# yhtang/GraphDot

Measured on AMD Instinct MI355X. Metric: graph-pairs/sec (Gram matrix), higher is better.
Workload: dtype f64

## Files before the change

graphdot_amd/csrc/device/mgk_oc.h:

```cpp
#ifndef GRAPHDOT_HIP_MGK_OC_H_
#define GRAPHDOT_HIP_MGK_OC_H_
#include "mgk_solver.h"

#ifdef GD_MARKS
#define GD_MARK(name) asm volatile("; GDMARK " #name)
#else
#define GD_MARK(name) ((void)0)
#endif

namespace graphdot {
namespace mgk {

template<int DMAX> struct class_order {
    constexpr static int NC = DMAX + 1, NCP = NC * NC;
    unsigned char d1[NCP], d2[NCP];
    constexpr class_order() : d1{}, d2{} {
        int n = 0;
        for (int p = DMAX * DMAX; p >= 0; --p)
            for (int a = 0; a <= DMAX; ++a)
                for (int b = 0; b <= DMAX; ++b)
                    if (a * b == p) {
                        d1[n] = (unsigned char)a;
                        d2[n] = (unsigned char)b;
                        ++n;
// ... 137 lines not shown
    constexpr static bool PK2 = DENSE && packed_edge<EdgeK>::value && sizeof(real) == 4;
    constexpr static int NR = R * T;
    constexpr static int NC = DMAX + 1;
    constexpr static int NCP = NC * NC;
    constexpr static int NTAB = ((NCP + 63) / 64) * 64;
    constexpr static int NM = S > 0 ? (S + 31) / 32 : 1;
    constexpr static int SETUP_CHUNK = 4;
    constexpr static bool ONE_PASS = sizeof(real) == 4 || W == 1;
    constexpr static int GCH = (STATIC && W == 1 && !NODAL && (sizeof(real) == 8 || C == 2)) ? 16 : 8;
    constexpr static bool ADDTID = W == 1 && C == 1 && sizeof(real) == 4 && !STATIC && !FLY;
    constexpr static bool PACK = C == 1 && !NODAL && !STATIC && !FLY &&
                                 (sizeof(real) == 4 ? (S >= 64 && W >= 8) : W >= 16);
    constexpr static int NADR = PACK ? (S + 1) / 2 : SA;
    constexpr static int lds_slot_count() {
        if (C != 1 || NODAL || NGRAD || STATIC || FLY || W == 1) return 0;
        if (sizeof(real) == 8 && W == 16 && (S == 40 || S == 64)) return 10;
        return 0;
    }
    constexpr static int SL = lds_slot_count();
    constexpr static int SREG = S - SL;
    constexpr static bool SEQ = C == 2 && STATIC && !NODAL && W == 1 && sizeof(real) == 8;
    constexpr static int CW = SEQ ? 1 : C;
    constexpr static bool LEAN = STATIC && C == 2 && !NODAL && !SEQ;
#ifndef GD_OC_FSCAL
#define GD_OC_FSCAL 1
#endif
    constexpr static bool FSCAL = GD_OC_FSCAL != 0 && sizeof(real) == 8 && !NGRAD;
    using sreal = std::conditional_t<FSCAL, float, real>;
    constexpr static int NSYS = C / CW;
    constexpr static bool DLDS = sizeof(real) == 8 && STATIC && W == 1 && C == 1 && !NODAL &&
                                 !NGRAD && !MAXIMIN && !FLY && R == 6;
    constexpr static bool HAS_Y = (!STATIC && !FLY) || LEAN || SEQ || DLDS;
    constexpr static int Y_REALS = DLDS ? 2 * R * 64 * W : R * 64 * W * C;
    template<class L> constexpr static int grid_slots() {
        if constexpr (L::is_static && !NGRAD) return L::T.end[0] == DMAX * DMAX ? DMAX * DMAX : 0;
        else return 0;
    }
    constexpr static int G0 = grid_slots<LAY>();
    static_assert(G0 == 0 || ONE_PASS, "the grid walk belongs to the one-pass slot setup");
    template<class L> constexpr static bool layout_matches() {
        if constexpr (L::is_static) return L::S == S && L::R == R;
        else return true;
    }
    static_assert(layout_matches<LAY>(), "the static layout must have S slots in R batches");
    template<class M> __device__ static __forceinline__ bool flush_at(int s, M const &m) {
        if constexpr (STATIC) return LAY::T.last[s];
        else return (m[s / 32] >> (s % 32)) & 1u;
    }
    constexpr static bool KEEP_X = NODAL || C == 2;
    constexpr static int n_jac = PStart::jac_dims + 1 + NodeK::jac_dims + EdgeK::jac_dims;
    constexpr static int off_q = PStart::jac_dims;
    constexpr static int off_v = off_q + 1;
    constexpr static int off_e = off_v + NodeK::jac_dims;
    constexpr static class_order<DMAX> ORD{};

    struct lds_t {
        real red[2][2 * W];
        int tab_off[NTAB];
        int tab_cls[64];
        unsigned mm_cell[4];
    };

    __device__ static __forceinline__ int uni(int v) { return __builtin_amdgcn_readfirstlane(v); }

    template<class V> __device__ static __forceinline__ V scalar_load(V const *ptr) {
        static_assert(sizeof(V) % 4 == 0, "whole dwords");
        typedef const unsigned __attribute__((address_space(4))) *const_words;
        const_words w = (const_words)(std::uintptr_t)ptr;
        unsigned buf[sizeof(V) / 4];
#pragma unroll
        for (unsigned k = 0; k < sizeof(V) / 4; ++k) buf[k] = w[k];
// ... 2 lines not shown
        return out;
    }

    __device__ static __forceinline__ graph_header_t load_header(graph_header_t const *ptr, [[maybe_unused]] int &n_orig) {
        if constexpr (QUOT) {
            graph_header_t h = scalar_load(ptr);
            n_orig = (int)((unsigned)h.n_node >> 16);
            h.n_node &= 0xFFFF;
            return h;
        } else {
            return scalar_load(ptr);
        }
    }
    __device__ static __forceinline__ Graph view_graph(char const *image, graph_header_t const &h, [[maybe_unused]] int n_orig) {
        if constexpr (QUOT) return Graph::quotient(image, h, n_orig);
        else return Graph(image, h);
    }

    __device__ static __forceinline__ float cg_ratio(float a, float b) { return a / b; }
    __device__ static __forceinline__ double cg_ratio(double a, double b) {
        double y = __builtin_amdgcn_rcp(b);
        y = __builtin_fma(__builtin_fma(-b, y, 1.0), y, y);
        y = __builtin_fma(__builtin_fma(-b, y, 1.0), y, y);
        return a * y;
    }

    __device__ static __forceinline__ int row_pos(int k, int wv, int lane) {
        return k * T + 64 * ((k & 1) ? W - 1 - wv : wv) + lane;
    }

    struct row_t {
        int i1, i2, rs1, rs2, d1, d2, prod;
    };
    constexpr static int GD_ = G0 ? DMAX : 1;
    constexpr static int GQ_ = QUOT ? GD_ : 1;
    struct grid_t {
        unsigned a[GD_], b[GD_];
        unsigned j1[GD_], j2[GD_];
        unsigned t1[GD_], t2[GD_];
        bool u[GD_], v[GD_];
        int row;
    };

    __device__ static __forceinline__ void run(PF const &full, lds_t &lds, real *dyn) {
        P const &prm = common(full);
        const int lane = wave::laneid();
        const int tid = (W == 1) ? lane : (int)threadIdx.x;
        const int wv = (W == 1) ? 0 : uni((int)(threadIdx.x / 64));
        real *const lp = dyn;
        real *const lY = lp + (size_t)prm.u_capacity * C;
        unsigned *const rowmap = reinterpret_cast<unsigned *>(lY + (HAS_Y ? (size_t)Y_REALS : (size_t)0));
        char *const lG1 = reinterpret_cast<char *>(rowmap + NR);
        char *const lG2 = lG1 + prm.g_capacity;
        [[maybe_unused]] real *const lV = reinterpret_cast<real *>(lG2 + prm.g_capacity);
        real *const red0 = lds.red[0], *const red1 = lds.red[1];
        using reduce = alternating_reduce<real, W>;
        using sreduce = alternating_reduce<sreal, W>;
        sreal *const sred0 = reinterpret_cast<sreal *>(red0), *const sred1 = reinterpret_cast<sreal *>(red1);
        const unsigned lY_off = uni((int)lds_offset(lY));
        graph_header_t const *const headers = reinterpret_cast<graph_header_t const *>(prm.arena);
        const int dump = (int)prm.u_capacity - 1;

        if constexpr (DENSE) {
            if (prm.flags & F_DENSE) {
                for (unsigned k = tid; k < prm.u_capacity * (unsigned)C; k += T) lp[k] = real(0);
                job_sync<W>();
            }
        }
        for (unsigned t = blockIdx.x; t < prm.n_launch_jobs; t += gridDim.x) {
            const job_t job = scalar_load(prm.jobs + t);
            [[maybe_unused]] int no1 = 0, no2 = 0;
            const graph_header_t h1 = load_header(headers + job.i, no1), h2 = load_header(headers + job.j, no2);
            const int n1 = h1.n_node, n2 = h2.n_node, N = n1 * n2;
            const int ldp = n2 | 1;
            const real q = prm.q, q0 = prm.q0;
            const real inv1q2 = real(1) / ((real(1) - q) * (real(1) - q));
            const real bscale = q * q / (q0 * q0);
            const unsigned nzpad1 = ((unsigned)n1 + 3u) & ~3u, nzpad2 = ((unsigned)n2 + 3u) & ~3u;
            const unsigned cb1 = TAB ? (nzpad1 + (((unsigned)h1.n_nz + 3u) & ~3u) + 15u) & ~15u : 0u;
            const unsigned cb2 = TAB ? (nzpad2 + (((unsigned)h2.n_nz + 3u) & ~3u) + 15u) & ~15u : 0u;

            GD_MARK(stage);
            job_sync<W>();
            {
                typedef unsigned v4 __attribute__((ext_vector_type(4)));
                const unsigned w1 = (h1.perm + 2u * n1 - h1.degree + cb1 + 15u) / 16u;
                const unsigned w2 = (h2.perm + 2u * n2 - h2.degree + cb2 + 15u) / 16u;
                const v4 *const s1 = reinterpret_cast<const v4 *>(prm.arena + h1.degree - cb1);
                const v4 *const s2 = reinterpret_cast<const v4 *>(prm.arena + h2.degree - cb2);
                v4 *const d1 = reinterpret_cast<v4 *>(lG1);
                v4 *const d2 = reinterpret_cast<v4 *>(lG2);
                constexpr int K = 2;
                const unsigned wmax = w1 > w2 ? w1 : w2;
#pragma nounroll
                for (unsigned base = 0; base < wmax; base += K * T) {
                    v4 v1[K], v2[K];
#pragma unroll
                    for (int k = 0; k < K; ++k) {
                        const unsigned w = base + k * T + tid;
                        v1[k] = w < w1 ? s1[w] : v4{0u, 0u, 0u, 0u};
                        v2[k] = w < w2 ? s2[w] : v4{0u, 0u, 0u, 0u};
                    }
#pragma unroll
                    for (int k = 0; k < K; ++k) {
                        const unsigned w = base + k * T + tid;
// ... 133 lines not shown

            struct walk_t {
                unsigned e1, end1, last1, e2, rs2, end2;
                int row;
                __device__ __forceinline__ bool valid() const { return e1 < end1; }
                __device__ __forceinline__ unsigned a() const { return e1 < last1 ? e1 : last1; }
                __device__ __forceinline__ void next() {
                    ++e2;
                    const bool wrap = e2 == end2;
                    e2 = wrap ? rs2 : e2;
                    e1 += wrap ? 1u : 0u;
                }
            };
            auto open_walk = [&](int kb) -> walk_t {
                const row_t r = open_row(kb);
                const bool live = r.prod > 0;
                walk_t w;
                w.e1 = live ? (unsigned)r.rs1 : 0u;
                w.end1 = live ? (unsigned)(r.rs1 + r.d1) : 0u;
                w.last1 = live ? (unsigned)(r.rs1 + r.d1 - 1) : 0u;
                w.rs2 = live ? (unsigned)r.rs2 : 0u;
                w.end2 = live ? (unsigned)(r.rs2 + r.d2) : 1u;
                w.e2 = w.rs2;
                w.row = r.i1 * ldp + r.i2;
                return w;
            };

            auto open_grid = [&](unsigned base, unsigned elem) -> grid_t {
                const row_t r = open_row(0);
                const bool live = r.prod > 0;
                grid_t g;
                g.row = r.i1 * ldp + r.i2;
#pragma unroll
                for (int k = 0; k < GD_; ++k) {
                    g.u[k] = k < r.d1;
                    g.v[k] = k < r.d2;
                    g.a[k] = live ? (unsigned)r.rs1 + (g.u[k] ? (unsigned)k : 0u) : 0u;
                    g.b[k] = live ? (unsigned)r.rs2 + (g.v[k] ? (unsigned)k : 0u) : 0u;
                    const nz_t z1 = at32(g1.nz, g.a[k]), z2 = at32(g2.nz, g.b[k]);
                    g.j1[k] = base + __umul24((unsigned)z1.j, (unsigned)ldp) * elem;
                    g.j2[k] = (unsigned)z2.j * elem;
                    if constexpr (TAB) {
                        g.t1[k] = __umul24((unsigned)ecls1[g.a[k]], nec);
                        g.t2[k] = (unsigned)ecls2[g.b[k]];
                    }
                }
                return g;
            };

            GD_MARK(slots);
            real val[SA];
            unsigned adr[NADR];
            const unsigned lp_off = lds_offset(lp);
            constexpr unsigned ELEM = CW * sizeof(real);
            unsigned fm[NM];
#pragma unroll
            for (int w = 0; w < NM; ++w) fm[w] = 0;
            int n_slots = 0;
            if constexpr (!FLY) {
                if constexpr (STATIC) {
#pragma unroll
                    for (int k = 0; k < R; ++k)
                        if (k * T < N) n_slots = LAY::T.end[k];
                } else {
#pragma unroll
                for (int k = 0; k < R; ++k) {
                    const int pos = row_pos(k, wv, 0);
                    int trip = 0;
                    if (pos < N) {
                        const unsigned rm = (unsigned)uni((int)rowmap[pos]);
                        const int i1 = (int)(rm >> 16), i2 = (int)(rm & 0xFFFFu);
                        trip = uni(((int)lrp1[i1 + 1] - (int)lrp1[i1]) * ((int)lrp2[i2 + 1] - (int)lrp2[i2]));
                    }
                    if (trip > 0) {
                        n_slots += trip;
                        const int last = n_slots - 1;
#pragma unroll
                        for (int w = 0; w < NM; ++w)
                            if (last / 32 == w) fm[w] |= 1u << (last % 32);
                    }
                }
                n_slots = n_slots > S ? S : n_slots;
                }
                if constexpr (ONE_PASS) {
                    int kb = 0;
                    walk_t cur = G0 ? walk_t{} : open_walk(0);
                    [[maybe_unused]] grid_t grid;
                    [[maybe_unused]] edge_t ge1[GD_], ge2[GD_];
                    [[maybe_unused]] real gw1[GQ_], gw2[GQ_];
                    if constexpr (G0 > 0) {
                        grid = open_grid(lp_off, ELEM);
                        if constexpr (QUOT) {
#pragma unroll
                            for (int k = 0; k < GD_; ++k) {
                                gw1[k] = qweight(g1, at32(g1.nz, grid.a[k]));
                                gw2[k] = qweight(g2, at32(g2.nz, grid.b[k]));
                            }
                        }
                        if constexpr (!TAB || (GD_WEIGHTED && edge_weight<edge_t>::value)) {
#pragma unroll
                            for (int k = 0; k < GD_; ++k) {
                                ge1[k] = at32(g1.edge, grid.a[k]);
                                ge2[k] = at32(g2.edge, grid.b[k]);
                            }
                        }
                    }
    #pragma unroll
                    for (int s = 0; s < S; ++s) {
                        if (s % SETUP_CHUNK == 0) __builtin_amdgcn_sched_barrier(0);
                        real e;
                        bool ok;
                        unsigned col;
                        if (s < G0) {
                            const int gu = s / GD_, gv = s % GD_;
                            ok = grid.u[gu] && grid.v[gv];
                            if constexpr (TAB) {
                                e = at32(ketab, grid.t1[gu] + grid.t2[gv]);
                                if constexpr (GD_WEIGHTED && edge_weight<edge_t>::value)
                                    e *= real(edge_weight<edge_t>::get(ge1[gu])) *
                                         real(edge_weight<edge_t>::get(ge2[gv]));
                            } else {
                                e = prm.edge_kernel(ge1[gu], ge2[gv]);
                            }
                            if constexpr (QUOT) e *= gw1[gu] * gw2[gv];
                            col = ok ? grid.j1[gu] + grid.j2[gv] : lp_off;
                        } else {
                        ok = cur.valid();
                        const unsigned a = cur.a(), b = cur.e2;
                        const nz_t z1 = at32(g1.nz, a), z2 = at32(g2.nz, b);
                        if constexpr (TAB) {
                            e = at32(ketab, __umul24((unsigned)ecls1[a], nec) + ecls2[b]);
                            if constexpr (GD_WEIGHTED && edge_weight<edge_t>::value)
                                e *= real(edge_weight<edge_t>::get(at32(g1.edge, a))) *
                                     real(edge_weight<edge_t>::get(at32(g2.edge, b)));
                        } else {
                            const edge_t e1 = at32(g1.edge, a), e2 = at32(g2.edge, b);
                            e = prm.edge_kernel(e1, e2);
                        }
                        if constexpr (QUOT) e *= qweight(g1, z1) * qweight(g2, z2);
                        col = ok ? __umul24((unsigned)z1.j, (unsigned)ldp) + (unsigned)z2.j : 0u;
                        col = lp_off + col * ELEM;
                        }
                        if (SL > 0 && s >= SREG) {
                            lV[(s - SREG) * T + tid] = ok ? e : real(0);
                        } else {
                            val[s] = ok ? e : real(0);
                        }
// ... 1084 lines not shown
                                const unsigned col = (unsigned)at32(g2.nz, b).j;
                                real w = w1 * load_real_at<real>(rowp + col * ELEM);
                                if constexpr (TAB) {
                                    const unsigned cidx = c1 + ecls2[b];
                                    if constexpr (GD_WEIGHTED && edge_weight<edge_t>::value)
                                        w *= real(edge_weight<edge_t>::get(at32(g2.edge, b)));
#pragma unroll
                                    for (int jj = 0; jj < EdgeK::jac_dims; ++jj)
                                        jac[off_e + jj] += w * at32(dketab, (unsigned)jj * nec * nec + cidx);
                                } else {
                                    auto de = prm.edge_kernel._j_a_c_o_b_i_a_n_(e1, at32(g2.edge, b));
#pragma unroll
                                    for (int jj = 0; jj < EdgeK::jac_dims; ++jj) jac[off_e + jj] += w * real(de[jj]);
                                }
                            }
                        }
                    }
                } else if constexpr (EdgeK::jac_dims > 0) {
                    int kb = 0;
                    walk_t cur = G0 ? walk_t{} : open_walk(0);
                    [[maybe_unused]] grid_t grid;
                    if constexpr (G0 > 0) {
                        grid = open_grid(0u, 0u);
                        cur.row = grid.row;
                    }
                    auto yp_of = [&](int row) -> real {
                        if constexpr (SEQ) return lp[(unsigned)prm.u_capacity + (unsigned)row];
                        else return lp[row * 2 + 1];
                    };
                    real yrow = yp_of(cur.row);
#pragma unroll
                    for (int s = 0; s < S; ++s) {
                        if (s < n_slots) {
                            const bool ok = s < G0 ? grid.u[s / GD_] && grid.v[s % GD_] : cur.valid();
                            const unsigned a = s < G0 ? grid.a[s / GD_] : cur.a();
                            const unsigned b = s < G0 ? grid.b[s % GD_] : cur.e2;
                            real w = ok ? yrow * load_real_at<real>(adr[s]) : real(0);
                            if constexpr (TAB) {
                                const unsigned cidx = __umul24((unsigned)ecls1[a], nec) + ecls2[b];
                                if constexpr (GD_WEIGHTED && edge_weight<edge_t>::value)
                                    w *= real(edge_weight<edge_t>::get(g1.edge[a])) *
                                         real(edge_weight<edge_t>::get(g2.edge[b]));
#pragma unroll
                                for (int jj = 0; jj < EdgeK::jac_dims; ++jj)
                                    jac[off_e + jj] += w * at32(dketab, (unsigned)jj * nec * nec + cidx);
                            } else {
                                const edge_t e1 = g1.edge[a], e2 = g2.edge[b];
                                auto de = prm.edge_kernel._j_a_c_o_b_i_a_n_(e1, e2);
#pragma unroll
                                for (int jj = 0; jj < EdgeK::jac_dims; ++jj) jac[off_e + jj] += w * real(de[jj]);
                            }
                            if (s >= G0) cur.next();
                            if (flush_at(s, fm) && s != S - 1) {
                                ++kb;
                                cur = open_walk(kb);
                                yrow = yp_of(cur.row);
                            }
                        }
                    }
                }
#pragma unroll
                for (int j = 0; j < n_jac; ++j) {
                    const real g = reduce::sum(jac[j], (j & 1) ? red1 : red0);
                    if (tid == 0) {
                        if (flags & F_PACKED) {
                            prm.gradient[(size_t)prm.order[t] * n_jac + j] = g;
                        } else if (flags & F_DIAGONAL) {
                            prm.gradient[(size_t)I1 + (size_t)prm.nX * j] = g;
                        } else {
// ... 38 lines not shown
```

graphdot_amd/csrc/gdhost.cpp:

```cpp
#include "gdhost.h"
#include "gdquotient.h"

#include <algorithm>
#include <cstdlib>
#include <cstring>
#include <numeric>
#include <atomic>
#include <cmath>
#include <exception>
#include <mutex>
#include <thread>
#include <vector>

namespace {

constexpr int64_t ALIGN = 16;
inline int64_t pad(int64_t n) { return (n + ALIGN - 1) / ALIGN * ALIGN; }

struct rect_order_t {
    int a[256], b[256], prod[257];
    int n_upto[16], upto[16][256];
    rect_order_t() {
        int n = 0;
        for (int p = 15 * 15; p >= 0; --p)
// ... 418 lines not shown
        int prods[256], nr = 0;
        {
            const uint16_t *h1 = hist + (size_t)a * 16, *h2 = hist + (size_t)b * 16;
            int64_t c = 0;
            for (int u = 0; u < RECT.n_upto[pmd]; ++u) {
                const int k = RECT.upto[pmd][u];
                const int64_t sz = (int64_t)h1[RECT.a[k]] * h2[RECT.b[k]];
                if (sz == 0) continue;
                c += sz;
                cum[nr] = c;
                prods[nr] = RECT.prod[k];
                ++nr;
            }
        }
        auto trip_at = [&](int64_t first) -> int {
            if (first >= N) return 0;
            int k = 0;
            while (k < nr && cum[k] <= first) ++k;
            return k < nr ? prods[k] : 0;
        };
        int trips1[MAXL + 1];
        {
            int k = 0;
            for (int bt = 0; bt <= MAXL; ++bt) {
                const int64_t first = 64 * (int64_t)bt;
                while (k < nr && cum[k] <= first) ++k;
                trips1[bt] = (first < N && k < nr) ? prods[k] : 0;
            }
        }
        for (int32_t v = 0; v < n_var; ++v) {
            const bool fly = S[v] == 0;
            if (!fly && (pmd_true > D[v] || pmd_true > 14)) continue;
            const int64_t T = 64 * (int64_t)W[v];
            if (N > T * R[v] || np_ >= (fly ? 0x3FFF : 0xFFFF)) continue;
            const int64_t NR = T * R[v];
            const int64_t pcap = (np_ + 1 + 3) / 4 * 4;
            const int64_t NRy = ((n_L[v] > 0 && C != 2) || fly) ? 0 : NR;
            const int64_t lds = (pcap + NRy) * C * real_size + 4 * NR + 2 * gbytes +
                                4 * (int64_t)W[v] * real_size + 4 * (D[v] > 6 ? 128 : 64) + 256 + 16 +
                                (extra_lds ? extra_lds[v] : 0);
            if (lds > lds_limit) continue;
            const int64_t nb = (N + T - 1) / T;
            bool ok = true;
            if (fly) {
                ok = pmd_true > fly_min_degree;
            } else if (n_L[v] > 0) {
                for (int64_t k = 0; k < nb && ok; ++k) {
                    const int cap = k < n_L[v] && k < MAXL ? L[(size_t)v * MAXL + k] : 0;
                    ok = (W[v] == 1 && k <= MAXL ? trips1[k] : trip_at(k * T)) <= cap;
                }
            } else if (W[v] == 1 && nb <= MAXL + 1) {
                int64_t total = 0;
                for (int64_t k = 0; k < nb; ++k) total += trips1[k];
                ok = total <= S[v];
            } else {
                int64_t worst = 0;
                for (int32_t wv = 0; wv < W[v]; ++wv) {
                    int64_t total = 0;
                    for (int64_t k = 0; k < nb; ++k)
                        total += trip_at(k * T + 64 * ((k & 1) ? W[v] - 1 - wv : wv));
                    worst = std::max(worst, total);
                }
                ok = worst <= S[v];
            }
            if (ok) {
                choice[t] = v;
                break;
            }
        }
// ... 146 lines not shown
```

graphdot_amd/kernel/marginalized/_backend_hip.py:

```python
import copy
import os
import re
import uuid
import zlib
from collections import OrderedDict, namedtuple
import numpy as np
from ...codegen import Template
from ...util import gcpause
from ...util.cookie import IdentityCache
from ...codegen.sympy_printer import to_real_expr
from ...codegen.typetool import _dtype_util
from ...hip import jit, runtime
from ...microkernel import TensorProduct, Product
from ...util.iterable import flatten, fold_like
from ._backend import Backend
from ._devicegraph import (DeviceGraph, GraphArena, HIST_BINS, class_bytes,
                           degree_histograms, graph_features, pack_many,
                           quotient_graph)

_TEMPLATE = os.path.join(os.path.dirname(__file__), 'template.hip')

F_NODAL, F_DIAGONAL, F_SYMMETRIC, F_LMIN1, F_BLOCK, F_PACKED, F_REFCOMPAT, \
    F_DENSE = 1, 2, 4, 8, 16, 32, 64, 128

# ... 9 lines not shown
def stream_parts(costs, count, resident, queued):
    if costs is None or len(costs) == 0:
        return max(1, min(resident // max(count, 1), STREAM_MAX_PARTS))
    c = np.asarray(costs, dtype=np.float64)
    best, best_t = 1, max(c[0], c.sum() / max(1, min(resident, queued)))
    table = dict(STREAM_PART_EFFICIENCY)
    ms, es = zip(*STREAM_PART_EFFICIENCY)
    own = min(resident // max(len(c), 1), STREAM_MAX_PARTS)
    for M in sorted(set(ms[1:]) | ({own} if own > 1 else set())):
        if M > min(resident, STREAM_MAX_PARTS):
            break
        eff = table.get(M) or float(np.interp(np.log2(M), np.log2(ms), es))
        groups = max(1, resident // M)
        pad = -len(c) % groups
        load = np.concatenate((c, np.zeros(pad))).reshape(-1, groups).sum(0)
        t = load.max() / (M * eff)
        if t < 0.95 * best_t:
            best, best_t = M, t
    return best


def OCStatic(*L, D=4):
    return OCVariant(1, int(sum(L)), len(L), D, tuple(int(x) for x in L))


VARIANTS = [
    Variant(1, 8, 2), Variant(1, 12, 3), Variant(1, 16, 4), Variant(1, 20, 5),
    Variant(1, 24, 6), Variant(1, 28, 7), Variant(1, 32, 9), Variant(1, 48, 9),
    Variant(1, 64, 16),
    Variant(4, 16, 4), Variant(4, 32, 8), Variant(4, 64, 16),
    Variant(16, 16, 2), Variant(16, 32, 4), Variant(16, 64, 8),
    Variant(16, 128, 16),
]
OC_STATIC_VARIANTS = [
    OCStatic(16), OCStatic(16, 4), OCStatic(16, 4, 1), OCStatic(16, 4, 4),
    OCStatic(16, 4, 4, 1), OCStatic(16, 4, 4, 1, 1), OCStatic(16, 4, 4, 3, 1),
    OCStatic(16, 4, 4, 3, 1, 1), OCStatic(16, 4, 4, 4, 1, 1, 1),
    OCStatic(16, 4, 4, 4, 3, 1, 1, 1), OCStatic(16, 4, 4, 4, 4, 1, 1, 1, 1),
]
OC_FLY_VARIANTS = [
    OCVariant(4, 0, 1, 0), OCVariant(4, 0, 2, 0), OCVariant(4, 0, 3, 0),
    OCVariant(8, 0, 2, 0), OCVariant(16, 0, 2, 0), OCVariant(16, 0, 4, 0),
]
OC_VARIANTS = OC_STATIC_VARIANTS + [
    OCVariant(1, 12, 2, 4), OCVariant(1, 16, 3, 4), OCVariant(1, 20, 3, 4),
    OCVariant(1, 20, 4, 4), OCVariant(1, 24, 4, 4), OCVariant(1, 28, 5, 4),
    OCVariant(1, 28, 6, 4), OCVariant(1, 32, 7, 4), OCVariant(1, 36, 9, 4),
    OCVariant(1, 32, 3, 8), OCVariant(1, 48, 5, 8), OCVariant(1, 64, 9, 8),
    OCVariant(4, 32, 3, 8), OCVariant(4, 40, 2, 8), OCVariant(4, 48, 4, 8),
    OCVariant(4, 64, 5, 8),
    OCVariant(8, 40, 2, 8), OCVariant(8, 48, 3, 8), OCVariant(8, 64, 4, 8),
    OCVariant(16, 32, 2, 8), OCVariant(16, 40, 2, 8), OCVariant(16, 48, 3, 8),
    OCVariant(16, 64, 3, 8),
] + OC_FLY_VARIANTS
FLY_MIN_DEGREE = 8
GENERAL = Variant(0, 0, 0)
TABLES = Variant(-1, 0, 0)
GENERAL_THREADS = 1024
MFMA = Variant(-3, 0, 0)
MFMA_MAX_NODES = 32
STREAM = Variant(-2, 0, 0)
STREAM_THREADS = 1024
STREAM_ROWS = {4: 8, 8: 8}
STREAM_CAP = 16
STREAM_MAX_PARTS = 256
STREAM_LDS_BUDGET = 159 * 1024
LDS_LIMIT = 160 * 1024
_LARGE_PAIR_SOLVERS = [MFMA, STREAM, GENERAL]
# ... 556 lines not shown

    def waves_per_eu(self, v, C):
        floor = -(-64 * v.W * (WPB1 if v.W == 1 else 1) // 256)
        if self.occupancy is not None and (v.W, v.S) in self.occupancy:
            return max(self.occupancy[(v.W, v.S)], floor)
        if isinstance(v, OCVariant):
            return max(self._oc_waves(v, C), -(-64 * v.W // 256))
        if v.W == 1:
            f64 = np.dtype(self.real) == np.float64
            table = {(1, False): self._WAVES_F32_VALUE,
                     (2, False): self._WAVES_F32_GRADIENT,
                     (1, True): self._WAVES_F64_VALUE,
                     (2, True): self._WAVES_F64_GRADIENT}.get((C, f64), {})
            if v.S in table:
                return max(table[v.S], floor)
        if C == 1:
            w4 = self._WAVES_F32_VALUE_W4 \
                if np.dtype(self.real) == np.float32 \
                else self._WAVES_F64_VALUE_W4
            if (v.W, v.S) in w4:
                return max(w4[(v.W, v.S)], floor)
        need = 5.3 * v.S + 4 * v.R + 6
        if C == 2:
            need = 1.6 * need
        if np.dtype(self.real) == np.float64:
            need = 1.8 * need
        for n in (8, 6, 5, 4, 3, 2):
            if need <= (512 // n) // 8 * 8 + 4:
                return max(n, floor)
        return max(1, floor)

    _OC_WAVES = {
        (False, 1): {('L', 16): 6, ('L', 16, 4): 6, ('L', 16, 4, 1): 5, ('L', 16, 4, 4): 5,
                     ('L', 16, 4, 4, 1): 3, ('L', 16, 4, 4, 1, 1): 3,
                     ('L', 16, 4, 4, 3, 1): 4, ('L', 16, 4, 4, 3, 1, 1): 4,
                     ('L', 16, 4, 4, 4, 1, 1, 1): 3,
                     ('L', 16, 4, 4, 4, 3, 1, 1, 1): 3,
                     ('L', 16, 4, 4, 4, 4, 1, 1, 1, 1): 3,
                     (1, 12, 2, 4): 6, (1, 16, 3, 4): 6, (1, 20, 3, 4): 6,
                     (1, 20, 4, 4): 4, (1, 24, 4, 4): 5, (1, 28, 5, 4): 4,
                     (1, 28, 6, 4): 4, (1, 32, 7, 4): 4, (1, 36, 9, 4): 2,
                     (1, 32, 3, 8): 2, (1, 48, 5, 8): 2, (1, 64, 9, 8): 2,
                     (4, 32, 3, 8): 4, (4, 40, 2, 8): 4, (4, 48, 4, 8): 2,
                     (4, 64, 5, 8): 3, (8, 40, 2, 8): 4, (8, 48, 3, 8): 4,
                     (8, 64, 4, 8): 4, (16, 32, 2, 8): 4, (16, 40, 2, 8): 4,
                     (16, 48, 3, 8): 4, (16, 64, 3, 8): 4},
        (True, 1): {('L', 16): 4, ('L', 16, 4): 4, ('L', 16, 4, 1): 3, ('L', 16, 4, 4): 3,
                    ('L', 16, 4, 4, 1): 3, ('L', 16, 4, 4, 1, 1): 3,
                    ('L', 16, 4, 4, 3, 1): 3, ('L', 16, 4, 4, 3, 1, 1): 3,
                    ('L', 16, 4, 4, 4, 1, 1, 1): 2,
                    ('L', 16, 4, 4, 4, 3, 1, 1, 1): 2,
                    ('L', 16, 4, 4, 4, 4, 1, 1, 1, 1): 2,
                    (1, 12, 2, 4): 4, (1, 16, 3, 4): 4, (1, 20, 3, 4): 4,
                    (1, 20, 4, 4): 3, (1, 24, 4, 4): 3, (1, 28, 5, 4): 3,
                    (1, 28, 6, 4): 3, (1, 32, 7, 4): 2, (1, 36, 9, 4): 2,
                    (1, 64, 9, 8): 1, (4, 32, 3, 8): 3, (4, 40, 2, 8): 3,
                    (4, 64, 5, 8): 2, (8, 40, 2, 8): 2, (8, 64, 4, 8): 2},
        (False, 2): {('L', 16): 4, ('L', 16, 4): 4, ('L', 16, 4, 1): 4, ('L', 16, 4, 4): 2,
                     ('L', 16, 4, 4, 1): 2, ('L', 16, 4, 4, 1, 1): 3,
                     ('L', 16, 4, 4, 3, 1): 3, ('L', 16, 4, 4, 3, 1, 1): 3,
                     ('L', 16, 4, 4, 4, 1, 1, 1): 2,
                     ('L', 16, 4, 4, 4, 3, 1, 1, 1): 2,
                     ('L', 16, 4, 4, 4, 4, 1, 1, 1, 1): 2,
                     (1, 12, 2, 4): 4, (1, 16, 3, 4): 4, (1, 20, 3, 4): 3,
                     (1, 20, 4, 4): 2, (1, 24, 4, 4): 3, (1, 28, 5, 4): 3,
                     (1, 28, 6, 4): 2, (1, 32, 7, 4): 2, (1, 36, 9, 4): 2},
        (True, 2): {('L', 16): 2, ('L', 16, 4): 2, ('L', 16, 4, 1): 3, ('L', 16, 4, 4): 2,
                    ('L', 16, 4, 4, 1): 3, ('L', 16, 4, 4, 1, 1): 2,
                    ('L', 16, 4, 4, 3, 1): 2, ('L', 16, 4, 4, 3, 1, 1): 2,
                    ('L', 16, 4, 4, 4, 1, 1, 1): 2,
                    ('L', 16, 4, 4, 4, 3, 1, 1, 1): 2,
                    ('L', 16, 4, 4, 4, 4, 1, 1, 1, 1): 1,
                    (1, 12, 2, 4): 3, (1, 16, 3, 4): 3, (1, 20, 3, 4): 3,
                    (1, 20, 4, 4): 2, (1, 24, 4, 4): 2, (1, 28, 5, 4): 2,
                    (1, 28, 6, 4): 2, (1, 32, 7, 4): 2, (1, 36, 9, 4): 2},
    }

    _STATIC_OFF = {}

    def _static_enabled(self, v, C):
        f64 = np.dtype(self.real) == np.float64
        return v.L not in self._STATIC_OFF.get((f64, C), ())

    _FLY_WAVES = 3

    def _oc_waves(self, v, C, ngrad=False):
        f64 = np.dtype(self.real) == np.float64
        if v.S == 0:
            return max(self._FLY_WAVES, -(-64 * v.W // 256))
        hit = self._OC_WAVES.get((f64, C), {}).get(
            ('L',) + v.L if v.L else tuple(v)[:4])
        if hit and not ngrad:
            return hit
        w = 2 if f64 else 1
        need = (w * C + 1) * 0 + v.S * (w + 1) + v.R * (5 * w * C + 1) \
            + 8 * w * C + 24 + (6 * w * v.R if ngrad else 0)
        for n in (8, 6, 5, 4, 3, 2):
            if need <= (512 // n) // 8 * 8:
                return n
        return 1

    def _entry_point(self, v, C, nodal=False, tab=False, ngrad=False,
                     maximin=False, quot=False):
        if v == TABLES:
            return Template(r'''
extern "C" __global__ __launch_bounds__(256)
void ${name}(params_t prm) {
    graphdot::mgk::fill_tables<real_t, ${C}>(prm);
}
''').render(name=self.kernel_name(v, C), C=C)
        if isinstance(v, OCVariant):
            return Template(r'''
extern "C" __global__ __launch_bounds__(${threads})
__attribute__((amdgpu_waves_per_eu(${waves})))
void ${name}(${params} prm) {
# ... 305 lines not shown

    TRIP_BATCHES = 12

    def _degree_hists(self, dgraphs, maxdeg, D, hists):
        if D not in hists:
            h = np.zeros((len(dgraphs), D + 1), dtype=np.int64)
            for g_, dg_ in enumerate(dgraphs):
                if maxdeg[g_] <= D:
                    h[g_] = np.bincount(dg_.adjacency_count, minlength=D + 1)
            H, hid = np.unique(h, axis=0, return_inverse=True)
            hists[D] = (H, hid.reshape(-1))
        return hists[D]

    def _trip_table(self, ji, jj, dgraphs, maxdeg, pair_maxdeg, D, hists):
        H, hid = self._degree_hists(dgraphs, maxdeg, D, hists)
        nH = len(H)
        row = np.full(len(ji), -1, dtype=np.int64)
        idx = np.flatnonzero(pair_maxdeg <= D)
        pk = hid[ji[idx]] * nH + hid[jj[idx]]
        upk, inv = np.unique(pk, return_inverse=True)
        row[idx] = inv.reshape(-1)
        tr = self.oc_trips(H[upk // nH], H[upk % nH], D, self.TRIP_BATCHES)
        return tr, row

    def _classify_pairs(self, ji, jj, dgraphs, C, tab_bytes=0, gtab=False,
                        oc_only=False, nodal=False, mfma=False):
        f = graph_features(dgraphs)
        n_node, n_nz = f['n_node'], f['n_nz']
        deg_sorted = None
        n1, n2 = n_node[ji], n_node[jj]
        nnz1 = n_nz[ji]
        N = n1 * n2
        NP = n1 * (n2 | 1)
        cost = n_nz[ji] * n_nz[jj] + 4 * N
        choice = np.full(len(ji), -1, dtype=np.int64)
        slots = {}
        ntask = np.maximum((nnz1 + 1) * n2, n1 + n2 + 2)
        image = f['image_bytes']
        if tab_bytes:
            image = image + class_bytes(n_node, n_nz)
        gbytes = np.maximum(image[ji], image[jj])
        image_oc = image + class_bytes(n_node, n_nz) if gtab else image
        gbytes_oc = np.maximum(image_oc[ji], image_oc[jj])
        maxdeg = f['max_degree']
        pair_maxdeg = np.maximum(maxdeg[ji], maxdeg[jj])
        oc_slots, hists, trips = {}, {}, {}
        fly_off = False
        rem = np.arange(len(ji))
        is_oc = [isinstance(v, OCVariant) for v in self.variants]
        n_oc = sum(is_oc)
        native_oc = (self.native and not tab_bytes and n_oc > 0
                     and all(is_oc[:n_oc]) and len(ji) > 0
                     and len(dgraphs) < 2**31)
        if native_oc:
            from ...hip import hostlib
            menu = [(k, v) for k, v in enumerate(self.variants[:n_oc])
                    if (not v.L or self._static_enabled(v, C))
                    and (v.S > 0 or not fly_off)]
            hist = f['hist']
            ch, _ = hostlib.classify_oc(
                ji, jj, n_node, n_nz, image_oc, maxdeg, hist,
                [(v.W, v.S, v.R, v.D, v.L) for _, v in menu], C,
                np.dtype(self.real).itemsize, LDS_LIMIT, FLY_MIN_DEGREE,
                [self.lds_slot_bytes(v, C, nodal) for _, v in menu])
            idx = np.array([k for k, _ in menu], dtype=np.int64)
            hit = ch >= 0
            choice[hit] = idx[ch[hit]]
            rem = rem[~hit]
        for k, v in enumerate(self.variants):
            if not len(rem):
                break
            if v in (GENERAL, STREAM, MFMA) or (
                    oc_only and not isinstance(v, OCVariant)):
                continue
            if isinstance(v, OCVariant):
                if tab_bytes or native_oc:
                    continue
                if v.L and not self._static_enabled(v, C):
                    continue
                if v.S == 0:
                    if fly_off:
                        continue
                    fits = (N[rem] <= 64 * v.W * v.R) & (NP[rem] < 0x3FFF) \
                        & (pair_maxdeg[rem] > FLY_MIN_DEGREE)
                    fits &= self.lds_bytes(v, C, NP[rem], gbytes_oc[rem],
                                           nodal=nodal) <= LDS_LIMIT
                    choice[rem[fits]] = k
                    rem = rem[~fits]
                    continue
                fits = ((pair_maxdeg[rem] <= v.D) & (N[rem] <= 64 * v.W * v.R)
                        & (NP[rem] < 0xFFFF))
                if not fits.any():
                    continue
                fits &= self.lds_bytes(v, C, NP[rem], gbytes_oc[rem],
                                       nodal=nodal) <= LDS_LIMIT
                if v.L:
                    if v.D not in trips:
                        trips[v.D] = self._trip_table(
                            ji, jj, dgraphs, maxdeg, pair_maxdeg, v.D, hists)
                    tr, row = trips[v.D]
                    idx = rem[fits]
                    ok = row[idx] >= 0
                    L = np.zeros(tr.shape[1], dtype=np.int64)
                    L[:v.R] = v.L
                    ok[ok] = (tr[row[idx[ok]]] <= L[None, :]).all(axis=1)
                    choice[idx[ok]] = k
                    fits[fits] = ok
                    rem = rem[~fits]
                    continue
                if (v.W, v.D) not in oc_slots:
                    H, hid = self._degree_hists(dgraphs, maxdeg, v.D, hists)
                    idx = rem[pair_maxdeg[rem] <= v.D]
                    pk = hid[ji[idx]] * len(H) + hid[jj[idx]]
                    seen = np.zeros(len(H) * len(H), dtype=bool)
                    seen[pk] = True
                    upk = np.flatnonzero(seen)
                    lut = np.zeros(len(H) * len(H), dtype=np.int64)
                    lut[upk] = self.oc_slots_needed(
                        H[upk // len(H)], H[upk % len(H)], v.W, v.D)
                    sl = np.full(len(ji), np.iinfo(np.int64).max,
                                 dtype=np.int64)
                    sl[idx] = lut[pk]
                    oc_slots[(v.W, v.D)] = sl
                fits &= oc_slots[(v.W, v.D)][rem] <= v.S
                choice[rem[fits]] = k
                rem = rem[~fits]
                continue
            fits = (NP[rem] <= 64 * v.W * v.R) & (NP[rem] <= 0xFFFF)
            if not fits.any():
                continue
            fits &= self.lds_bytes(v, C, ntask[rem], gbytes[rem], tab_bytes) \
                <= LDS_LIMIT
            if v.W not in slots:
                if deg_sorted is None:
                    deg_sorted = np.zeros((len(dgraphs), int(n_node.max())),
                                          dtype=np.int64)
                    for k_, g in enumerate(dgraphs):
                        deg_sorted[k_, :g.n_node] = g.adjacency_count
# ... 5 lines not shown
            choice[rem[fits]] = k
            rem = rem[~fits]
        if mfma and MFMA in self.variants and C == 1 and not oc_only:
            dense = (n1 <= MFMA_MAX_NODES) & (n2 <= MFMA_MAX_NODES) & \
                (23 * n_nz[ji] * n_nz[jj] > 9 * N * N)
            choice[dense] = self.variants.index(MFMA)
            gbytes = np.where(dense, np.maximum(f['image_bytes'][ji],
                                                f['image_bytes'][jj]), gbytes)
        if np.any(choice < 0) and oc_only:
            raise NotOwnerComputes
        if np.any(choice < 0):
            if GENERAL not in self.variants:
                bad = int(np.argmax(choice < 0))
                raise NotImplementedError(
                    f'graph pair ({ji[bad]}, {jj[bad]}) with '
                    f'{n1[bad]}x{n2[bad]} nodes and {nnz1[bad]}x'
                    f'{n_nz[jj[bad]]} adjacency nonzeros exceeds the largest '
                    'register-resident solver variant and the general '
                    'solver is disabled')
            left = choice < 0
            choice[left] = self.variants.index(GENERAL)
            if STREAM in self.variants:
                raw = f['image_bytes']
                nv = np.zeros(len(dgraphs), dtype=np.int64)
                for g_ in np.unique(np.concatenate((ji[left], jj[left]))):
                    nv[g_] = self.stream_virtual_rows(
                        dgraphs[g_].adjacency_count) \
                        if n_node[g_] <= STREAM_THREADS else 0
                sb = self.stream_lds_bytes(raw[ji], raw[jj], n1, n2,
                                           nv[ji], nv[jj])
                fits = left & (sb + 1024 <= LDS_LIMIT)
                choice[fits] = self.variants.index(STREAM)
                gbytes = np.where(fits, sb, gbytes)
        return choice, cost, ntask, gbytes, NP, gbytes_oc, np.maximum(n1, n2)

    def _graphs_and_kernels(self, graphs, node_kernel, edge_kernel, traits,
                            timer=None, ngrad=False):
        tic = timer.tic if timer else (lambda *_: None)
        toc = timer.toc if timer else (lambda *_: None)
        tic('transferring graphs to GPU')
        if not isinstance(graphs, (list, tuple)):
            graphs = list(graphs)
        ckey, dgraphs = self._dgraph_lists.get(graphs)
        if dgraphs is None:
            key = (self.uuid.int, np.dtype(self.real).str)
            new = [g for g in graphs if key not in g.cookie]
            if new:
                for g, dg in zip(new, pack_many(new, real=self.real,
                                                native=self.native)):
                    g.cookie[key] = dg
            dgraphs = _DeviceGraphList(g.cookie[key] for g in graphs)
            sig0 = dgraphs[0].signature
            for dg in dgraphs:
                if dg.signature != sig0:
                    self._assert_homogeneous(dgraphs[0], dg)
            dgraphs.ids = tuple(map(id, dgraphs))
            self._dgraph_lists.put(ckey, graphs, dgraphs)
        toc('transferring graphs to GPU')
        if traits.eval_gradient is True and traits.nodal is not False \
                and not ngrad:
            raise NotImplementedError(
                'nodal gradients are evaluated by finite differences over '
                'value launches (HIPBackend._nodal_gradient), not by a '
                'gradient plan')
        C = 2 if traits.eval_gradient is True and not ngrad else 1
        fields = (self._used_fields(node_kernel),
# ... 37 lines not shown
    def _quotient_launches(launches):
        return all(isinstance(L['variant'], OCVariant) and L['variant'].S > 0
                   for L in launches)

    def _partition(self, dgraphs, jobs, C, tab_bytes=0, gtab=False,
                   oc_only=False, merge_map=None, nodal=False, mfma=False):
        jobs = np.ascontiguousarray(jobs)
        jobs_sorted = None
        sel, (choice, cost, ntask, gbytes, NP, gbytes_oc, nmax) = \
            self._classify_classes(None, None, dgraphs, C, tab_bytes, gtab,
                                   oc_only, jobs=jobs, nodal=nodal, mfma=mfma)
        applied = {}
        if merge_map is not None:
            for k, k2 in merge_map.items():
                choice = np.where(choice == k, k2, choice)
            applied = dict(merge_map)
        elif self.min_launch > 0:
            members_ = np.ones(len(choice), dtype=np.int64) if sel is None \
                else sel.members
            used_ = sorted(set(choice.tolist()))
            for a_, k in enumerate(used_):
                v = self.variants[k]
                if not isinstance(v, OCVariant):
                    continue
                here = choice == k
                if int(members_[here].sum()) * v.W >= self.min_launch:
                    continue
                for k2 in used_[a_ + 1:]:
                    v2 = self.variants[k2]
                    if not (isinstance(v2, OCVariant) and v2.W == v.W
                            and v2.D == v.D and v2.S >= v.S and v2.R >= v.R):
                        continue
                    if v2.L and not (v.L and all(
                            a <= b for a, b in zip(v.L, v2.L))):
                        continue
                    if True:
                        choice = np.where(here, k2, choice)
                        for k0, k1 in list(applied.items()):
                            if k1 == k:
                                applied[k0] = k2
                        applied[k] = k2
                        break
        choice = self._fit_launches_into_lds(choice, C, NP, ntask, gbytes,
                                             gbytes_oc, tab_bytes, oc_only,
                                             nodal)
        rank_of = np.empty(len(choice), dtype=np.int64)
        by_rank = np.lexsort((-cost, choice))
        step = np.ones(len(choice), dtype=np.int64)
        step[1:] = (choice[by_rank[1:]] != choice[by_rank[:-1]]) | \
            (cost[by_rank[1:]] != cost[by_rank[:-1]])
        rank_of[by_rank] = np.cumsum(step) - 1
        if sel is None:
            order_all = by_rank.astype(np.uint32)
            members = np.ones(len(choice), dtype=np.int64)
        elif self.native:
            from ...hip import hostlib
            rank_of_key = np.full(sel.nc * sel.nc, -1, dtype=np.int32)
            rank_of_key[sel.upk] = rank_of
            order_all, jobs_sorted = hostlib.order_jobs(
                sel.pk, rank_of_key, int(rank_of.max()) + 1, jobs)
            members = sel.members
        else:
            rank = rank_of[sel.sel]
            rank = rank.astype(np.uint16 if len(choice) <= 0xFFFF
                               else np.uint32)
            order_all = np.argsort(rank, kind='stable').astype(np.uint32)
            members = sel.members
        used = sorted(set(choice.tolist()))
        rsize = np.dtype(self.real).itemsize
        launches, cursor = [], 0
        for k in used:
            v = self.variants[k]
            idx = np.flatnonzero(choice == k)
            count = int(members[idx].sum())
            if v == GENERAL:
# ... 743 lines not shown
```

Before: 225.0 million.

## Add rectangular grid static layouts with role swapping for quotient graphs

Adds static OC layouts whose leading batch forms a D x (D-1) or (D-1) x (D-1) grid instead of only D x D, plus new variants (12,3), (16,3) and their tails. When one graph has higher degrees than the narrow side allows, the kernel swaps the two graphs' roles per job, and the host and Python selectors size the product buffer for either orientation. The intent is to drop unused grid slots for degree-limited pairs, cutting slot work and register use. In exchange it adds more variants to compile and dispatch, a larger product buffer for swapped cases, and extra selection logic.

```diff
diff --git a/graphdot_amd/csrc/device/mgk_oc.h b/graphdot_amd/csrc/device/mgk_oc.h
--- a/graphdot_amd/csrc/device/mgk_oc.h
+++ b/graphdot_amd/csrc/device/mgk_oc.h
@@ -193,11 +193,24 @@
                                  !NGRAD && !MAXIMIN && !FLY && R == 6;
     constexpr static bool HAS_Y = (!STATIC && !FLY) || LEAN || SEQ || DLDS;
     constexpr static int Y_REALS = DLDS ? 2 * R * 64 * W : R * 64 * W * C;
+    constexpr static bool ROLES_FREE = QUOT && !NODAL && !MAXIMIN && !NGRAD && C == 1;
+    template<class L> constexpr static int grid_rows() {
+        if constexpr (L::is_static && !NGRAD && DMAX > 1) {
+            if (L::T.end[0] == DMAX * DMAX) return DMAX;
+            if (L::T.end[0] == DMAX * (DMAX - 1)) return ROLES_FREE ? DMAX : 0;
+            if (L::T.end[0] == (DMAX - 1) * (DMAX - 1)) return DMAX - 1;
+        }
+        return 0;
+    }
     template<class L> constexpr static int grid_slots() {
-        if constexpr (L::is_static && !NGRAD) return L::T.end[0] == DMAX * DMAX ? DMAX * DMAX : 0;
+        if constexpr (L::is_static) return grid_rows<L>() ? L::T.end[0] : 0;
         else return 0;
     }
     constexpr static int G0 = grid_slots<LAY>();
+    constexpr static int GU = G0 ? grid_rows<LAY>() : 1;
+    constexpr static int GV = G0 ? G0 / GU : 1;
+    constexpr static bool ORIENT = GU != GV;
+    static_assert(!ORIENT || ROLES_FREE, "swapped roles: graph-level values of quotient images only");
     static_assert(G0 == 0 || ONE_PASS, "the grid walk belongs to the one-pass slot setup");
     template<class L> constexpr static bool layout_matches() {
         if constexpr (L::is_static) return L::S == S && L::R == R;
@@ -266,13 +279,12 @@
     struct row_t {
         int i1, i2, rs1, rs2, d1, d2, prod;
     };
-    constexpr static int GD_ = G0 ? DMAX : 1;
-    constexpr static int GQ_ = QUOT ? GD_ : 1;
+    constexpr static int GQU = QUOT ? GU : 1, GQV = QUOT ? GV : 1;
     struct grid_t {
-        unsigned a[GD_], b[GD_];
-        unsigned j1[GD_], j2[GD_];
-        unsigned t1[GD_], t2[GD_];
-        bool u[GD_], v[GD_];
+        unsigned a[GU], b[GV];
+        unsigned j1[GU], j2[GV];
+        unsigned t1[GU], t2[GV];
+        bool u[GU], v[GV];
         int row;
     };
 
@@ -304,7 +316,20 @@
         for (unsigned t = blockIdx.x; t < prm.n_launch_jobs; t += gridDim.x) {
             const job_t job = scalar_load(prm.jobs + t);
             [[maybe_unused]] int no1 = 0, no2 = 0;
-            const graph_header_t h1 = load_header(headers + job.i, no1), h2 = load_header(headers + job.j, no2);
+            graph_header_t h1 = load_header(headers + job.i, no1), h2 = load_header(headers + job.j, no2);
+            if constexpr (ORIENT) {
+                bool flip = false;
+#pragma unroll
+                for (int d = GV + 1; d <= DMAX; ++d) flip |= h2.hist[d] != 0;
+                if (flip) {
+                    const graph_header_t h = h1;
+                    h1 = h2;
+                    h2 = h;
+                    const int no = no1;
+                    no1 = no2;
+                    no2 = no;
+                }
+            }
             const int n1 = h1.n_node, n2 = h2.n_node, N = n1 * n2;
             const int ldp = n2 | 1;
             const real q = prm.q, q0 = prm.q0;
@@ -504,17 +529,17 @@
                 grid_t g;
                 g.row = r.i1 * ldp + r.i2;
 #pragma unroll
-                for (int k = 0; k < GD_; ++k) {
+                for (int k = 0; k < GU; ++k) {
                     g.u[k] = k < r.d1;
-                    g.v[k] = k < r.d2;
+                    if (k < GV) g.v[k] = k < r.d2;
                     g.a[k] = live ? (unsigned)r.rs1 + (g.u[k] ? (unsigned)k : 0u) : 0u;
-                    g.b[k] = live ? (unsigned)r.rs2 + (g.v[k] ? (unsigned)k : 0u) : 0u;
-                    const nz_t z1 = at32(g1.nz, g.a[k]), z2 = at32(g2.nz, g.b[k]);
+                    if (k < GV) g.b[k] = live ? (unsigned)r.rs2 + (g.v[k] ? (unsigned)k : 0u) : 0u;
+                    const nz_t z1 = at32(g1.nz, g.a[k]), z2 = at32(g2.nz, k < GV ? g.b[k] : 0u);
                     g.j1[k] = base + __umul24((unsigned)z1.j, (unsigned)ldp) * elem;
-                    g.j2[k] = (unsigned)z2.j * elem;
+                    if (k < GV) g.j2[k] = (unsigned)z2.j * elem;
                     if constexpr (TAB) {
                         g.t1[k] = __umul24((unsigned)ecls1[g.a[k]], nec);
-                        g.t2[k] = (unsigned)ecls2[g.b[k]];
+                        if (k < GV) g.t2[k] = (unsigned)ecls2[g.b[k]];
                     }
                 }
                 return g;
@@ -558,22 +583,22 @@
                     int kb = 0;
                     walk_t cur = G0 ? walk_t{} : open_walk(0);
                     [[maybe_unused]] grid_t grid;
-                    [[maybe_unused]] edge_t ge1[GD_], ge2[GD_];
-                    [[maybe_unused]] real gw1[GQ_], gw2[GQ_];
+                    [[maybe_unused]] edge_t ge1[GU], ge2[GV];
+                    [[maybe_unused]] real gw1[GQU], gw2[GQV];
                     if constexpr (G0 > 0) {
                         grid = open_grid(lp_off, ELEM);
                         if constexpr (QUOT) {
 #pragma unroll
-                            for (int k = 0; k < GD_; ++k) {
+                            for (int k = 0; k < GU; ++k) {
                                 gw1[k] = qweight(g1, at32(g1.nz, grid.a[k]));
-                                gw2[k] = qweight(g2, at32(g2.nz, grid.b[k]));
+                                if (k < GV) gw2[k] = qweight(g2, at32(g2.nz, grid.b[k]));
                             }
                         }
                         if constexpr (!TAB || (GD_WEIGHTED && edge_weight<edge_t>::value)) {
 #pragma unroll
-                            for (int k = 0; k < GD_; ++k) {
+                            for (int k = 0; k < GU; ++k) {
                                 ge1[k] = at32(g1.edge, grid.a[k]);
-                                ge2[k] = at32(g2.edge, grid.b[k]);
+                                if (k < GV) ge2[k] = at32(g2.edge, grid.b[k]);
                             }
                         }
                     }
@@ -584,7 +609,7 @@
                         bool ok;
                         unsigned col;
                         if (s < G0) {
-                            const int gu = s / GD_, gv = s % GD_;
+                            const int gu = s / GV, gv = s % GV;
                             ok = grid.u[gu] && grid.v[gv];
                             if constexpr (TAB) {
                                 e = at32(ketab, grid.t1[gu] + grid.t2[gv]);
@@ -1735,9 +1760,9 @@
 #pragma unroll
                     for (int s = 0; s < S; ++s) {
                         if (s < n_slots) {
-                            const bool ok = s < G0 ? grid.u[s / GD_] && grid.v[s % GD_] : cur.valid();
-                            const unsigned a = s < G0 ? grid.a[s / GD_] : cur.a();
-                            const unsigned b = s < G0 ? grid.b[s % GD_] : cur.e2;
+                            const bool ok = s < G0 ? grid.u[s / GV] && grid.v[s % GV] : cur.valid();
+                            const unsigned a = s < G0 ? grid.a[s / GV] : cur.a();
+                            const unsigned b = s < G0 ? grid.b[s % GV] : cur.e2;
                             real w = ok ? yrow * load_real_at<real>(adr[s]) : real(0);
                             if constexpr (TAB) {
                                 const unsigned cidx = __umul24((unsigned)ecls1[a], nec) + ecls2[b];
diff --git a/graphdot_amd/csrc/gdhost.cpp b/graphdot_amd/csrc/gdhost.cpp
--- a/graphdot_amd/csrc/gdhost.cpp
+++ b/graphdot_amd/csrc/gdhost.cpp
@@ -474,9 +474,18 @@
             const bool fly = S[v] == 0;
             if (!fly && (pmd_true > D[v] || pmd_true > 14)) continue;
             const int64_t T = 64 * (int64_t)W[v];
-            if (N > T * R[v] || np_ >= (fly ? 0x3FFF : 0xFFFF)) continue;
+            int gu = 0, gv = 0;
+            if (n_L[v] > 0 && D[v] > 1) {
+                const int l0 = L[(size_t)v * MAXL], d = D[v];
+                if (l0 == d * d) gu = gv = d;
+                else if (l0 == d * (d - 1)) gu = d, gv = d - 1;
+                else if (l0 == (d - 1) * (d - 1)) gu = gv = d - 1;
+            }
+            const int64_t np_v = gu != gv ? std::max(np_, n2 * (n1 | 1)) : np_;
+            if (N > T * R[v] || np_v >= (fly ? 0x3FFF : 0xFFFF)) continue;
+            if (gu && (pmd_true > gu || std::min(maxdeg[a], maxdeg[b]) > gv)) continue;
             const int64_t NR = T * R[v];
-            const int64_t pcap = (np_ + 1 + 3) / 4 * 4;
+            const int64_t pcap = (np_v + 1 + 3) / 4 * 4;
             const int64_t NRy = ((n_L[v] > 0 && C != 2) || fly) ? 0 : NR;
             const int64_t lds = (pcap + NRy) * C * real_size + 4 * NR + 2 * gbytes +
                                 4 * (int64_t)W[v] * real_size + 4 * (D[v] > 6 ? 128 : 64) + 256 + 16 +
diff --git a/graphdot_amd/kernel/marginalized/_backend_hip.py b/graphdot_amd/kernel/marginalized/_backend_hip.py
--- a/graphdot_amd/kernel/marginalized/_backend_hip.py
+++ b/graphdot_amd/kernel/marginalized/_backend_hip.py
@@ -65,8 +65,10 @@
     Variant(16, 16, 2), Variant(16, 32, 4), Variant(16, 64, 8),
     Variant(16, 128, 16),
 ]
+OC_QUOTIENT_LAYOUTS = ((12, 3), (16, 3), (12, 3, 1), (16, 3, 1))
 OC_STATIC_VARIANTS = [
-    OCStatic(16), OCStatic(16, 4), OCStatic(16, 4, 1), OCStatic(16, 4, 4),
+    OCStatic(12, 3), OCStatic(16), OCStatic(16, 3), OCStatic(16, 4),
+    OCStatic(12, 3, 1), OCStatic(16, 3, 1), OCStatic(16, 4, 1), OCStatic(16, 4, 4),
     OCStatic(16, 4, 4, 1), OCStatic(16, 4, 4, 1, 1), OCStatic(16, 4, 4, 3, 1),
     OCStatic(16, 4, 4, 3, 1, 1), OCStatic(16, 4, 4, 4, 1, 1, 1),
     OCStatic(16, 4, 4, 4, 3, 1, 1, 1), OCStatic(16, 4, 4, 4, 4, 1, 1, 1, 1),
@@ -689,6 +691,7 @@
 
     _OC_WAVES = {
         (False, 1): {('L', 16): 6, ('L', 16, 4): 6, ('L', 16, 4, 1): 5, ('L', 16, 4, 4): 5,
+                     ('L', 12, 3): 6, ('L', 16, 3): 6, ('L', 12, 3, 1): 5, ('L', 16, 3, 1): 5,
                      ('L', 16, 4, 4, 1): 3, ('L', 16, 4, 4, 1, 1): 3,
                      ('L', 16, 4, 4, 3, 1): 4, ('L', 16, 4, 4, 3, 1, 1): 4,
                      ('L', 16, 4, 4, 4, 1, 1, 1): 3,
@@ -703,6 +706,7 @@
                      (8, 64, 4, 8): 4, (16, 32, 2, 8): 4, (16, 40, 2, 8): 4,
                      (16, 48, 3, 8): 4, (16, 64, 3, 8): 4},
         (True, 1): {('L', 16): 4, ('L', 16, 4): 4, ('L', 16, 4, 1): 3, ('L', 16, 4, 4): 3,
+                    ('L', 12, 3): 4, ('L', 16, 3): 4, ('L', 12, 3, 1): 3, ('L', 16, 3, 1): 3,
                     ('L', 16, 4, 4, 1): 3, ('L', 16, 4, 4, 1, 1): 3,
                     ('L', 16, 4, 4, 3, 1): 3, ('L', 16, 4, 4, 3, 1, 1): 3,
                     ('L', 16, 4, 4, 4, 1, 1, 1): 2,
@@ -735,9 +739,37 @@
 
     _STATIC_OFF = {}
 
-    def _static_enabled(self, v, C):
+    def _static_enabled(self, v, C, quot=True):
         f64 = np.dtype(self.real) == np.float64
+        if v.L in OC_QUOTIENT_LAYOUTS and not quot:
+            return False
         return v.L not in self._STATIC_OFF.get((f64, C), ())
+
+    @staticmethod
+    def grid_of(L, D):
+        if not L or D < 2:
+            return None
+        if L[0] in (D * D, D * (D - 1)):
+            return D, L[0] // D
+        if L[0] == (D - 1) * (D - 1):
+            return D - 1, D - 1
+        return None
+
+    @classmethod
+    def swaps_roles(cls, v, maxdeg_j):
+        g = cls.grid_of(v.L, v.D) if isinstance(v, OCVariant) else None
+        maxdeg_j = np.asarray(maxdeg_j)
+        if g is None or g[0] == g[1]:
+            return np.zeros(maxdeg_j.shape, dtype=bool)
+        return maxdeg_j > g[1]
+
+    @classmethod
+    def _grid_takes(cls, v2, v):
+        g2 = cls.grid_of(v2.L, v2.D)
+        if g2 is None or g2 == (v2.D, v2.D):
+            return True
+        g = cls.grid_of(v.L, v.D)
+        return g is not None and g[0] <= g2[0] and g[1] <= g2[1]
 
     _FLY_WAVES = 3
 
@@ -1109,6 +1141,11 @@
         nnz1 = n_nz[ji]
         N = n1 * n2
         NP = n1 * (n2 | 1)
+        NP_either = np.maximum(NP, n2 * (n1 | 1))
+
+        def rows_of(v):
+            g = self.grid_of(v.L, v.D) if isinstance(v, OCVariant) else None
+            return NP_either if g is not None and g[0] != g[1] else NP
         cost = n_nz[ji] * n_nz[jj] + 4 * N
         choice = np.full(len(ji), -1, dtype=np.int64)
         slots = {}
@@ -1126,14 +1163,24 @@
         rem = np.arange(len(ji))
         is_oc = [isinstance(v, OCVariant) for v in self.variants]
         n_oc = sum(is_oc)
+        quot = bool(C == 1 and not nodal and len(dgraphs) and
+                    getattr(dgraphs[0], 'n_orig', None) is not None)
+
+        def grid_fits(v, idx):
+            g = self.grid_of(v.L, v.D)
+            if g is None:
+                return np.ones(len(idx), dtype=bool)
+            a, b = maxdeg[ji[idx]], maxdeg[jj[idx]]
+            return (np.maximum(a, b) <= g[0]) & (np.minimum(a, b) <= g[1])
+        menu = [(k, v) for k, v in enumerate(self.variants[:n_oc])
+                if isinstance(v, OCVariant)
+                and (not v.L or self._static_enabled(v, C, quot))
+                and (v.S > 0 or not fly_off)]
         native_oc = (self.native and not tab_bytes and n_oc > 0
                      and all(is_oc[:n_oc]) and len(ji) > 0
                      and len(dgraphs) < 2**31)
         if native_oc:
             from ...hip import hostlib
-            menu = [(k, v) for k, v in enumerate(self.variants[:n_oc])
-                    if (not v.L or self._static_enabled(v, C))
-                    and (v.S > 0 or not fly_off)]
             hist = f['hist']
             ch, _ = hostlib.classify_oc(
                 ji, jj, n_node, n_nz, image_oc, maxdeg, hist,
@@ -1153,7 +1200,7 @@
             if isinstance(v, OCVariant):
                 if tab_bytes or native_oc:
                     continue
-                if v.L and not self._static_enabled(v, C):
+                if v.L and not self._static_enabled(v, C, quot):
                     continue
                 if v.S == 0:
                     if fly_off:
@@ -1165,11 +1212,12 @@
                     choice[rem[fits]] = k
                     rem = rem[~fits]
                     continue
+                NPv = rows_of(v)
                 fits = ((pair_maxdeg[rem] <= v.D) & (N[rem] <= 64 * v.W * v.R)
-                        & (NP[rem] < 0xFFFF))
+                        & (NPv[rem] < 0xFFFF))
                 if not fits.any():
                     continue
-                fits &= self.lds_bytes(v, C, NP[rem], gbytes_oc[rem],
+                fits &= self.lds_bytes(v, C, NPv[rem], gbytes_oc[rem],
                                        nodal=nodal) <= LDS_LIMIT
                 if v.L:
                     if v.D not in trips:
@@ -1181,6 +1229,7 @@
                     L = np.zeros(tr.shape[1], dtype=np.int64)
                     L[:v.R] = v.L
                     ok[ok] = (tr[row[idx[ok]]] <= L[None, :]).all(axis=1)
+                    ok &= grid_fits(v, idx)
                     choice[idx[ok]] = k
                     fits[fits] = ok
                     rem = rem[~fits]
@@ -1252,6 +1301,9 @@
                 fits = left & (sb + 1024 <= LDS_LIMIT)
                 choice[fits] = self.variants.index(STREAM)
                 gbytes = np.where(fits, sb, gbytes)
+        for k in set(choice.tolist()):
+            if k >= 0 and rows_of(self.variants[k]) is NP_either:
+                NP = np.where(choice == k, NP_either, NP)
         return choice, cost, ntask, gbytes, NP, gbytes_oc, np.maximum(n1, n2)
 
     def _graphs_and_kernels(self, graphs, node_kernel, edge_kernel, traits,
@@ -1355,15 +1407,15 @@
                             and v2.D == v.D and v2.S >= v.S and v2.R >= v.R):
                         continue
                     if v2.L and not (v.L and all(
-                            a <= b for a, b in zip(v.L, v2.L))):
+                            a <= b for a, b in zip(v.L, v2.L))
+                            and self._grid_takes(v2, v)):
                         continue
-                    if True:
-                        choice = np.where(here, k2, choice)
-                        for k0, k1 in list(applied.items()):
-                            if k1 == k:
-                                applied[k0] = k2
-                        applied[k] = k2
-                        break
+                    choice = np.where(here, k2, choice)
+                    for k0, k1 in list(applied.items()):
+                        if k1 == k:
+                            applied[k0] = k2
+                    applied[k] = k2
+                    break
         choice = self._fit_launches_into_lds(choice, C, NP, ntask, gbytes,
                                              gbytes_oc, tab_bytes, oc_only,
                                              nodal)
```

Result: faster. 242.7 million (median of 6 runs) (+7.9%).
